# michael-fonder/M4Depth

Measured on AMD Instinct MI355X. Metric: frames/s, higher is better.
Workload: dtype f32

## Files before the change

### include/m4depth_hip.h

```cpp
#ifndef M4DEPTH_HIP_H_
#define M4DEPTH_HIP_H_

#include <stdint.h>

#ifdef __cplusplus
extern "C" {
#endif

#define M4D_ABI_VERSION 6

int m4d_abi_version(void);
long long m4d_launch_count(void);
const char* m4d_build_info(void);
const char* m4d_switches_info(void);


int m4d_backproject_fwd(const float* input, const float* coords, const int dims[6],
                        float* out, void* stream);

int m4d_backproject_bwd(const float* grad, const float* input, const float* coords,
                        const int dims[6], float* input_grad, float* coords_grad, void* stream);


int m4d_dense_image_warp(const float* image, const float* flow, int B, int H, int W, int C,
// ... 214 lines not shown
                    int b, int h, int w, int C, int nbre_cuts, int cv_accum,
                    float* f_input, int f_stride, float log_scale, void* stream);
int m4d_level_front_r(const float* raw_f, float* norm_out, const float* prev_f, const float* depth_prev_t,
                      const float* prev_l_parallax, const float* prev_l_other, int ph, int pw,
                      const float* rot, int rot_c, const float* trans, const float* cam_f, const float* cam_c,
                      int b, int h, int w, int C, int nbre_cuts, int dscv_range, int sncv_range, int cv_accum,
                      float* f_input, int f_stride, float log_scale, void* stream);

int m4d_camera_pyramid(const float* cam_f, const float* cam_c, int b, int levels, float* f_out, float* c_out,
                       void* stream);

int m4d_level_post(const float* refiner_out, const float* rot, int rot_c, const float* trans,
                   const float* cam_f, const float* cam_c, int b, int h, int w, float scale,
                   float* parallax, float* depth, float* other, float* depth_state, void* stream);

int m4d_bias_act(const float* x, const float* bias, long long rows, int C, float slope,
                 float* out, void* stream);

int m4d_bias_act_padded(const float* x, const float* bias, int b, int h, int w, int C, float slope,
                        float* out, int out_h, int out_w, int off_y, int off_x, void* stream);

int m4d_conv3x3_bias_act(const float* x, const float* wp, const float* bias, int b, int h, int w,
                         int Cin, int Cout, int CoutPad, float slope, float* out, void* stream);
long long m4d_conv3x3_workspace_floats(int b, int h, int w, int CoutPad);
int m4d_conv3x3s_bias_act_ws(const float* x, const float* wp, const float* bias, int b, int h, int w,
                             int Cin, int Cout, int CoutPad, int stride, float slope, float* out,
                             float* workspace, long long workspace_floats, void* stream);
int m4d_conv3x3_bias_act_ws(const float* x, const float* wp, const float* bias, int b, int h, int w,
                            int Cin, int Cout, int CoutPad, float slope, float* out, float* workspace,
                            long long workspace_floats, void* stream);
int m4d_conv3x3s_bias_act_wsb(const float* x, const float* wp, const float* bias, int b, int split_batch, int h, int w,
                              int Cin, int Cout, int CoutPad, int stride, float slope, float* out,
                              float* workspace, long long workspace_floats, void* stream);
int m4d_conv3x3_lat(const float* x, int s_in, long long x_slab_floats, const float* x_bias, float x_slope,
                    const void* wp, const float* bias, int b, int h, int w, int Cin, int Cout, float slope,
                    int mt, int kw, int s_out, float* out, long long out_slab_floats, void* stream);
int m4d_conv3x3s_lat(const float* x, int s_in, long long x_slab_floats, const float* x_bias, float x_slope,
                     const void* wp, const float* bias, int b, int h, int w, int Cin, int Cout, int stride, float slope,
                     int mt, int kw, int s_out, float* out, long long out_slab_floats, void* stream);
int m4d_conv3x3_lat_f16(const float* x, int s_in, long long x_slab_floats, const float* x_bias, float x_slope,
                        const void* wp, const float* bias, int b, int h, int w, int Cin, int Cout, float slope,
                        int mt, int kw, int s_out, float* out, long long out_slab_floats, void* stream);
int m4d_partial_finish(const float* x, int s_in, long long x_slab_floats, const float* bias, float slope,
                       long long pixels, int C, float* out, void* stream);

int m4d_conv3x3_small_bias_act(const float* x, const float* wp, const float* bias, int b, int h, int w,
                               int Cin, int Cout, int CoutPad, float slope, float* out, void* stream);
int m4d_conv3x3s_small_bias_act(const float* x, const float* wp, const float* bias, int b, int h, int w,
                                int Cin, int Cout, int CoutPad, int stride, float slope, float* out, void* stream);
int m4d_conv3x3_small6_bias_act(const float* x, const void* wp6, const float* bias, int b, int h, int w,
                                int Cin, int Cout, int CoutPad, float slope, float* out, void* stream);

long long m4d_dinl_workspace_floats(int b, int C);
int m4d_dinl_fwd_padded(const float* x, const float* scale, const float* bias, int b, int h, int w, int C,
                        float slope, float* workspace, float* out, int out_h, int out_w, int off_y,
                        int off_x, void* stream);
int m4d_dinl_fwd(const float* x, const float* scale, const float* bias, int b, int h, int w, int C,
                 float slope, float* workspace, float* out, void* stream);

int m4d_enc_level0_fwd(const float* images, int bsz, long long stride_b, long long stride_t,
                       const float* w1_hwio, const float* bias1, const float* dn_scale, const float* dn_bias,
                       float dn_slope, const float* w2_hwio, const float* bias2, float slope,
                       int b, int h, int w, float* workspace, float* out, void* stream);
int m4d_enc_level0_stats(const float* images, int bsz, long long stride_b, long long stride_t,
                         const float* w1_hwio, const float* bias1, int b, int h, int w, float* workspace,
                         float* mean, float* var, void* stream);
int m4d_enc_level0_apply(const float* images, int bsz, long long stride_b, long long stride_t,
                         const float* w1_hwio, const float* bias1, const float* mean, const float* var,
                         const float* dn_scale, const float* dn_bias, float dn_slope, const float* w2_hwio,
                         const float* bias2, float slope, int b, int h, int w, float* out, void* stream);
int m4d_enc_head_fwd(const float* images, int bsz, long long stride_b, long long stride_t,
                     const float* w_hwio, const float* bias, int b, int h, int w, int C,
                     float* workspace, float* raw_out, void* stream);
int m4d_conv3x3s2_dinl_bias_act(const float* x_raw, const float* mean, const float* var, const float* dn_scale,
                                const float* dn_bias, float dn_slope, const float* wp, const float* bias,
                                int b, int h, int w, int Cout, int CoutPad, float slope, float* out, void* stream);

long long m4d_metrics_workspace_bytes(void);
int m4d_depth_metrics(const float* gt, const float* est, long long n, float max_d, void* workspace,
                      float* out7, float* total7, float count, float* mean7, void* stream);
int m4d_depth_metrics_strided(const float* gt, long long per_image, long long gt_image_stride, const float* est,
                              long long n, float max_d, void* workspace, float* out7, float* total7, float count,
// ... 94 lines not shown
```

### m4depth_amd/csrc/m4d_conv.hip

```cpp
#include "m4d_common.h"
#include "../../include/m4depth_hip.h"

namespace {

typedef float f32x16 __attribute__((ext_vector_type(16)));

struct ConvArgs {
  const float* x; const float* wp; const float* bias; float* out;
  int b, h, w, Cin, Cout, CoutPad, n_chunks, tiles_x, tiles_y;
  int oh, ow, pad_y, pad_x;
  float slope;
  int ksplit, chunks_per_split;
  float* ws;
  const float* dn_mean; const float* dn_var; const float* dn_scale; const float* dn_bias; float dn_slope;
};

constexpr int kTW = 16, kTH = 8;
constexpr int kKC = 16, kRS = 20;

template <int NT, int TS, int STRIDE, bool DB, int MINB, bool DINL = false>
__global__ void __launch_bounds__(256, MINB)
conv3x3_mfma_kernel(const ConvArgs a) {
  constexpr int kHWT = (kTW - 1) * STRIDE + 3, kHHT = (kTH - 1) * STRIDE + 3, kHP = kHWT * kHHT;
  constexpr int BN = 32 * NT;
// ... 350 lines not shown
  __syncthreads();

  constexpr int kRP = 36;
  float* red = lds_dyn;
#pragma unroll
  for (int r = 0; r < 16; ++r) {
    const int mr = (r & 3) + 8 * (r >> 2) + 4 * kh;
    red[(wave * 32 + mr) * kRP + m] = acc[r];
  }
  __syncthreads();
  {
    const int p = t >> 3, cq = t & 7;
    const int oy = tile_y + (p >> 3), ox = tile_x + (p & 7);
    const int co = n0 + 4 * cq;
    if (oy < a.oh && ox < a.ow && co < a.Cout) {
      const float4 s0 = *reinterpret_cast<const float4*>(red + (0 * 32 + p) * kRP + 4 * cq);
      const float4 s1 = *reinterpret_cast<const float4*>(red + (1 * 32 + p) * kRP + 4 * cq);
      const float4 s2 = *reinterpret_cast<const float4*>(red + (2 * 32 + p) * kRP + 4 * cq);
      const float4 s3 = *reinterpret_cast<const float4*>(red + (3 * 32 + p) * kRP + 4 * cq);
      const float sum[4] = {((s0.x + s1.x) + s2.x) + s3.x, ((s0.y + s1.y) + s2.y) + s3.y,
                            ((s0.z + s1.z) + s2.z) + s3.z, ((s0.w + s1.w) + s2.w) + s3.w};
      float* op = a.out + (((long long)bi * a.oh + oy) * a.ow + ox) * a.Cout + co;
#pragma unroll
      for (int e = 0; e < 4; ++e) {
        if (co + e < a.Cout) {
          float v = sum[e] + a.bias[co + e];
          op[e] = v > 0.f ? v : v * a.slope;
        }
      }
    }
  }
}

typedef __bf16 s6_bf16x8 __attribute__((ext_vector_type(8)));
typedef __bf16 s6_bf16x2 __attribute__((ext_vector_type(2)));
constexpr int kS6Row = 24;
constexpr int kS6A = kSHP * kS6Row;
constexpr int kS6B = 9 * 32 * kS6Row;

__device__ __forceinline__ unsigned s6_pk(float a, float b) {
  s6_bf16x2 v; v[0] = (__bf16)a; v[1] = (__bf16)b;
  return __builtin_bit_cast(unsigned, v);
}

__global__ void __launch_bounds__(256, 1)
conv3x3_small6_kernel(const ConvArgs a) {
  constexpr int A_PER = (kSHP * 4 + 63) / 64;
  constexpr int B_PER = (9 * 32 * 6) / 64;
  extern __shared__ __align__(16) float lds_dyn[];
  const int t = threadIdx.x, lane = t & 63;
  const int wave = __builtin_amdgcn_readfirstlane(t >> 6);
  float* lds_a = lds_dyn + wave * (kS6A + kS6B);
  float* lds_b = lds_a + kS6A;
  const int tile = blockIdx.x;
  const int tile_y = (tile / a.tiles_x) * kSH, tile_x = (tile % a.tiles_x) * kSW;
  const int n0 = blockIdx.y * 32;
  const int bi = blockIdx.z;
  const float* ximg = a.x + (long long)bi * a.h * a.w * a.Cin;
  const unsigned char* wsplit = reinterpret_cast<const unsigned char*>(a.wp);

  int a_off[A_PER], a_dst[A_PER];
  unsigned a_ok = 0;
  const int aq = lane & 3;
#pragma unroll
  for (int u = 0; u < A_PER; ++u) {
    const int idx = u * 64 + lane;
// ... 149 lines not shown

template <int NT, int TS, int STRIDE, int MINB>
void launch_conv(const ConvArgs& a, dim3 grid, hipStream_t s) {
  constexpr bool DB = false;
  constexpr int HP = ((kTW - 1) * STRIDE + 3) * ((kTH - 1) * STRIDE + 3);
  constexpr size_t lds = (size_t)(HP * kRS + (DB ? 2 : 1) * TS * 32 * NT * kRS) * sizeof(float);
  if (lds > 64 * 1024) M4D_LDS_OPT_IN(&conv3x3_mfma_kernel<NT, TS, STRIDE, DB, MINB>);
  m4d_launch((conv3x3_mfma_kernel<NT, TS, STRIDE, DB, MINB>), grid, dim3(256), lds, s, a);
}

template <int STRIDE>
void dispatch_conv(const ConvArgs& a, int nt, dim3 grid, hipStream_t s) {
  const long long blocks = (long long)grid.x * grid.y * grid.z;
  constexpr long long occ3_min_blocks = 4 * 768;
  switch (nt) {
    case 4:
      if (STRIDE == 1 && blocks >= occ3_min_blocks) launch_conv<4, 3, STRIDE, STRIDE == 1 ? 3 : 1>(a, grid, s);
      else launch_conv<4, 3, STRIDE, STRIDE == 1 ? 2 : 1>(a, grid, s);
      break;
    case 3: launch_conv<3, 3, STRIDE, STRIDE == 1 ? 3 : 2>(a, grid, s); break;
    case 2: launch_conv<2, STRIDE == 1 ? 9 : 3, STRIDE, STRIDE == 1 ? 3 : 2>(a, grid, s); break;
    default: launch_conv<1, 9, STRIDE, STRIDE == 1 ? 4 : 2>(a, grid, s); break;
  }
}

}

extern "C" int m4d_conv3x3_bias_act(const float* x, const float* wp, const float* bias, int b, int h, int w,
                                    int Cin, int Cout, int CoutPad, float slope, float* out, void* stream) {
  return m4d_conv3x3s_bias_act_ws(x, wp, bias, b, h, w, Cin, Cout, CoutPad, 1, slope, out, nullptr, 0, stream);
}

static int launch_conv3x3_small(const float* x, const float* wp, const float* bias, int b, int h, int w, int Cin, int Cout,
                                int CoutPad, int stride, float slope, float* out, void* stream) {
  M4D_CHECK_ARG(x && wp && bias && out && b > 0 && h > 0 && w > 0 && Cout > 0 && (stride == 1 || stride == 2));
  M4D_CHECK_ARG(Cin >= 16 && Cin % 4 == 0 && CoutPad % 32 == 0 && CoutPad >= Cout);
  M4D_CHECK_ARG(((((uintptr_t)x) | ((uintptr_t)wp)) & 15u) == 0);
  ConvArgs a;
  a.x = x; a.wp = wp; a.bias = bias; a.out = out; a.b = b; a.h = h; a.w = w; a.Cin = Cin; a.Cout = Cout;
  a.CoutPad = CoutPad; a.n_chunks = (Cin + kKC - 1) / kKC;
  a.dn_mean = a.dn_var = a.dn_scale = a.dn_bias = nullptr; a.dn_slope = 1.0f;
  a.slope = slope;
  a.oh = (h + stride - 1) / stride; a.ow = (w + stride - 1) / stride;
  const int tot_y = (a.oh - 1) * stride + 3 - h, tot_x = (a.ow - 1) * stride + 3 - w;
  a.pad_y = (tot_y > 0 ? tot_y : 0) / 2; a.pad_x = (tot_x > 0 ? tot_x : 0) / 2;
  a.tiles_x = (a.ow + kSW - 1) / kSW; a.tiles_y = (a.oh + kSH - 1) / kSH;
  a.ksplit = 1; a.chunks_per_split = a.n_chunks; a.ws = nullptr;
  const int halo = ((kSW - 1) * stride + 3) * ((kSH - 1) * stride + 3);
  const size_t lds = (size_t)4 * (halo * kRS + kSB) * sizeof(float);
  if (stride == 1) M4D_LDS_OPT_IN(&conv3x3_small_kernel<1>);
  else M4D_LDS_OPT_IN(&conv3x3_small_kernel<2>);
  const dim3 grid((unsigned)(a.tiles_x * a.tiles_y), (unsigned)(CoutPad / 32), (unsigned)b);
  if (stride == 1) m4d_launch(conv3x3_small_kernel<1>, grid, dim3(256), lds, (hipStream_t)stream, a);
  else m4d_launch(conv3x3_small_kernel<2>, grid, dim3(256), lds, (hipStream_t)stream, a);
  return M4D_LAUNCH_RESULT();
}
extern "C" int m4d_conv3x3_small_bias_act(const float* x, const float* wp, const float* bias, int b, int h, int w,
                                          int Cin, int Cout, int CoutPad, float slope, float* out, void* stream) {
  return launch_conv3x3_small(x, wp, bias, b, h, w, Cin, Cout, CoutPad, 1, slope, out, stream);
}
extern "C" int m4d_conv3x3s_small_bias_act(const float* x, const float* wp, const float* bias, int b, int h, int w,
                                           int Cin, int Cout, int CoutPad, int stride, float slope, float* out, void* stream) {
  return launch_conv3x3_small(x, wp, bias, b, h, w, Cin, Cout, CoutPad, stride, slope, out, stream);
}

extern "C" int m4d_conv3x3_small6_bias_act(const float* x, const void* wp6, const float* bias, int b, int h, int w,
                                           int Cin, int Cout, int CoutPad, float slope, float* out, void* stream) {
  M4D_CHECK_ARG(x && wp6 && bias && out && b > 0 && h > 0 && w > 0 && Cout > 0);
  M4D_CHECK_ARG(Cin >= 16 && Cin % 4 == 0 && CoutPad % 32 == 0 && CoutPad >= Cout);
  M4D_CHECK_ARG(((((uintptr_t)x) | ((uintptr_t)wp6)) & 15u) == 0);
  ConvArgs a;
  a.x = x; a.wp = reinterpret_cast<const float*>(wp6); a.bias = bias; a.out = out; a.b = b; a.h = h; a.w = w; a.Cin = Cin; a.Cout = Cout;
  a.CoutPad = CoutPad; a.n_chunks = (Cin + kKC - 1) / kKC;
  a.dn_mean = a.dn_var = a.dn_scale = a.dn_bias = nullptr; a.dn_slope = 1.0f;
  a.oh = h; a.ow = w; a.pad_y = a.pad_x = 1; a.slope = slope;
  a.tiles_x = (w + kSW - 1) / kSW; a.tiles_y = (h + kSH - 1) / kSH;
  a.ksplit = 1; a.chunks_per_split = a.n_chunks; a.ws = nullptr;
  constexpr size_t lds = (size_t)4 * (kS6A + kS6B) * sizeof(float);
  M4D_LDS_OPT_IN(&conv3x3_small6_kernel);
  m4d_launch(conv3x3_small6_kernel, dim3((unsigned)(a.tiles_x * a.tiles_y), (unsigned)(CoutPad / 32), (unsigned)b), dim3(256),
                     lds, (hipStream_t)stream, a);
  return M4D_LAUNCH_RESULT();
}

extern "C" long long m4d_conv3x3_workspace_floats(int b, int h, int w, int CoutPad) {
  return 32LL * b * h * w * CoutPad;
}

extern "C" int m4d_conv3x3_bias_act_ws(const float* x, const float* wp, const float* bias, int b, int h, int w,
                                       int Cin, int Cout, int CoutPad, float slope, float* out, float* workspace,
                                       long long workspace_floats, void* stream) {
  return m4d_conv3x3s_bias_act_ws(x, wp, bias, b, h, w, Cin, Cout, CoutPad, 1, slope, out, workspace,
                                  workspace_floats, stream);
}

extern "C" int m4d_conv3x3s2_dinl_bias_act(const float* x_raw, const float* mean, const float* var, const float* dn_scale,
                                           const float* dn_bias, float dn_slope, const float* wp, const float* bias,
                                           int b, int h, int w, int Cout, int CoutPad, float slope, float* out, void* stream) {
  M4D_CHECK_ARG(x_raw && mean && var && dn_scale && dn_bias && wp && bias && out && b > 0 && h > 0 && w > 0 && Cout > 0);
  M4D_CHECK_ARG(CoutPad == 32 && Cout <= 32);
  M4D_CHECK_ARG(((((uintptr_t)x_raw) & 7u) == 0) && ((((uintptr_t)wp) & 15u) == 0));
  ConvArgs a;
  a.x = x_raw; a.wp = wp; a.bias = bias; a.out = out; a.b = b; a.h = h; a.w = w; a.Cin = 16; a.Cout = Cout;
  a.CoutPad = CoutPad; a.n_chunks = 1;
  a.oh = (h + 1) / 2; a.ow = (w + 1) / 2;
  const int tph = (a.oh - 1) * 2 + 3 - h, tpw = (a.ow - 1) * 2 + 3 - w;
  a.pad_y = (tph > 0 ? tph : 0) / 2; a.pad_x = (tpw > 0 ? tpw : 0) / 2;
  a.tiles_x = (a.ow + kTW - 1) / kTW; a.tiles_y = (a.oh + kTH - 1) / kTH; a.slope = slope;
  a.ksplit = 1; a.chunks_per_split = 1; a.ws = nullptr;
  a.dn_mean = mean; a.dn_var = var; a.dn_scale = dn_scale; a.dn_bias = dn_bias; a.dn_slope = dn_slope;
  constexpr int HP = ((kTW - 1) * 2 + 3) * ((kTH - 1) * 2 + 3);
  constexpr size_t lds = (size_t)(HP * kRS + 9 * 32 * kRS) * sizeof(float);
  if (lds > 64 * 1024) M4D_LDS_OPT_IN(&conv3x3_mfma_kernel<1, 9, 2, false, 2, true>);
  const dim3 grid((unsigned)(a.tiles_x * a.tiles_y), 1, (unsigned)b);
  m4d_launch((conv3x3_mfma_kernel<1, 9, 2, false, 2, true>), grid, dim3(256), lds, (hipStream_t)stream, a);
  return M4D_LAUNCH_RESULT();
}

extern "C" int m4d_conv3x3s_bias_act_wsb(const float* x, const float* wp, const float* bias, int b, int split_batch, int h,
                                         int w, int Cin, int Cout, int CoutPad, int stride, float slope, float* out,
                                         float* workspace, long long workspace_floats, void* stream);

extern "C" int m4d_conv3x3s_bias_act_ws(const float* x, const float* wp, const float* bias, int b, int h, int w,
                                        int Cin, int Cout, int CoutPad, int stride, float slope, float* out,
                                        float* workspace, long long workspace_floats, void* stream) {
  return m4d_conv3x3s_bias_act_wsb(x, wp, bias, b, b, h, w, Cin, Cout, CoutPad, stride, slope, out, workspace,
                                   workspace_floats, stream);
}

extern "C" int m4d_conv3x3s_bias_act_wsb(const float* x, const float* wp, const float* bias, int b, int split_batch, int h,
                                         int w, int Cin, int Cout, int CoutPad, int stride, float slope, float* out,
                                         float* workspace, long long workspace_floats, void* stream) {
  M4D_CHECK_ARG(x && wp && bias && out && b > 0 && split_batch > 0 && h > 0 && w > 0 && Cin > 0 && Cout > 0);
  M4D_CHECK_ARG((stride == 1 || stride == 2) && CoutPad % 32 == 0 && CoutPad >= Cout);
  M4D_CHECK_ARG(((((uintptr_t)x) & (Cin % 2 == 0 ? 7u : 3u)) == 0) && ((((uintptr_t)wp) & 15u) == 0));
  ConvArgs a;
  a.x = x; a.wp = wp; a.bias = bias; a.out = out; a.b = b; a.h = h; a.w = w; a.Cin = Cin; a.Cout = Cout;
  a.CoutPad = CoutPad; a.n_chunks = (Cin + kKC - 1) / kKC;
  a.dn_mean = a.dn_var = a.dn_scale = a.dn_bias = nullptr; a.dn_slope = 1.0f;
  a.oh = (h + stride - 1) / stride; a.ow = (w + stride - 1) / stride;
  const int tph = (a.oh - 1) * stride + 3 - h, tpw = (a.ow - 1) * stride + 3 - w;
  a.pad_y = (tph > 0 ? tph : 0) / 2; a.pad_x = (tpw > 0 ? tpw : 0) / 2;
  a.tiles_x = (a.ow + kTW - 1) / kTW; a.tiles_y = (a.oh + kTH - 1) / kTH; a.slope = slope;
  const long long tiles = (long long)a.tiles_x * a.tiles_y;
  const int n32 = CoutPad / 32;
  auto n_tiles_for = [&](int images) {
    int nt = n32 >= 4 && n32 % 4 == 0 ? 4 : (n32 % 3 == 0 ? 3 : (n32 % 2 == 0 ? 2 : 1));
    while (nt > 1 && tiles * images * (n32 / nt) < 512) nt = (nt == 4 || nt == 2) ? nt / 2 : 1;
    return nt;
  };
  const int nt = n_tiles_for(b);
  const long long blocks = tiles * split_batch * (n32 / n_tiles_for(split_batch));
  int ksplit = 1;
  constexpr int sk_target = 256, sk_min_chunks = 2, sk_max = 16;
  if (workspace != nullptr && blocks < 128 && a.n_chunks >= 4) {
    ksplit = (int)((sk_target + blocks - 1) / blocks);
    if (ksplit > a.n_chunks / sk_min_chunks) ksplit = a.n_chunks / sk_min_chunks;
    if (ksplit > sk_max) ksplit = sk_max;
    while (ksplit > 1 && (long long)ksplit * b * a.oh * a.ow * CoutPad > workspace_floats) --ksplit;
  }
  a.chunks_per_split = (a.n_chunks + ksplit - 1) / ksplit;
  ksplit = (a.n_chunks + a.chunks_per_split - 1) / a.chunks_per_split;
  a.ksplit = ksplit; a.ws = workspace;
  const dim3 grid((unsigned)tiles, (unsigned)(n32 / nt), (unsigned)(b * ksplit));
  hipStream_t s = (hipStream_t)stream;
  if (stride == 1) dispatch_conv<1>(a, nt, grid, s);
  else dispatch_conv<2>(a, nt, grid, s);
  if (ksplit > 1) {
    const long long pixels = (long long)b * a.oh * a.ow;
    long long g = (pixels * Cout + 255) / 256;
    if (g > 2048) g = 2048;
    m4d_launch(conv_splitk_reduce_kernel, dim3((unsigned)g), dim3(256), 0, s, workspace, bias, pixels, Cout,
                       CoutPad, ksplit, slope, out);
  }
  return M4D_LAUNCH_RESULT();
}
```

### m4depth_amd/network_ops.py

```python
from __future__ import annotations

import ctypes

import torch

from ._lib import lib, dptr, stream_ptr, check, as_f32
from .depth_operations import _CV_ACCUM


def normalize_cuts(x, nbre_cuts, out=None):
    x = as_f32(x, "x")
    b, h, w, C = x.shape
    if C % nbre_cuts != 0:
        raise ValueError(f"nbre_cuts={nbre_cuts} does not divide the {C} feature channels")
    if out is None:
        out = torch.empty_like(x)
    check(lib.m4d_normalize_cuts(dptr(x, "x"), b, h, w, C, int(nbre_cuts), dptr(out, "out"), stream_ptr()),
          "m4d_normalize_cuts")
    return out


def resize_bilinear_v1(x, out_h, out_w, mul=1.0):
    x = as_f32(x, "x")
    b, ih, iw, c = x.shape
    out = torch.empty((b, out_h, out_w, c), dtype=torch.float32, device=x.device)
    check(lib.m4d_resize_bilinear_v1(dptr(x, "x"), b, ih, iw, c, int(out_h), int(out_w), float(mul), dptr(out),
                                     stream_ptr()), "m4d_resize_bilinear_v1")
    return out


def resize_nearest(x, out_h, out_w, out=None):
    x = as_f32(x, "x")
    b, ih, iw, c = x.shape
    if out is None:
        out = torch.empty((b, out_h, out_w, c), dtype=torch.float32, device=x.device)
# ... 885 lines not shown
    est = as_f32(est, "est")
    b, h, w = est.shape[:3]
    if est.dim() != 4 or est.shape[3] != 1:
        raise ValueError(f"est: expected [b,h,w,1], got {tuple(est.shape)}")
    gs = _batch_stride(gt, "gt")
    if gt.shape[0] != b or gt.dim() not in (3, 4) or (gt.dim() == 4 and gt.shape[3] != 1):
        raise ValueError(f"gt {tuple(gt.shape)} is not the [b,H,W,1] ground truth of est {tuple(est.shape)}")
    H, W = gt.shape[1:3]
    if log.dim() != 2 or log.shape[1] != 2:
        raise ValueError(f"log: expected [rows, 2], got {tuple(log.shape)}")
    for name, t in (("counter", counter), ("first_bad", first_bad)):
        if not isinstance(t, torch.Tensor) or t.numel() != 1:
            raise ValueError(f"{name}: expected a one-element int64 device tensor")
    ws = _workspace("train_log", int(lib.m4d_train_log_workspace_bytes()), est.device)
    check(lib.m4d_train_log_step(dptr(loss.reshape(1), "loss"), ctypes.c_void_p(gt.data_ptr()), gs, dptr(est, "est"), b, H, W,
                                 h, w, dptr(log, "log"), log.shape[0], dptr(counter, "counter", torch.int64),
                                 dptr(first_bad, "first_bad", torch.int64), dptr(ws), stream_ptr()), "m4d_train_log_step")
    return log

def pack_conv_weights(kernel_hwio):
    import numpy as np
    k = np.asarray(kernel_hwio, dtype=np.float32)
    assert k.shape[:2] == (3, 3)
    cin, cout = k.shape[2], k.shape[3]
    nch = -(-cin // 16)
    cpad = -(-cout // 32) * 32
    full = np.zeros((3, 3, nch * 16, cpad), np.float32)
    full[:, :, :cin, :cout] = k
    perm = np.array([0, 2, 4, 6, 8, 10, 12, 14, 1, 3, 5, 7, 9, 11, 13, 15])
    w = full.reshape(9, nch, 16, cpad)[:, :, perm, :]
    return np.ascontiguousarray(w.transpose(1, 0, 3, 2)), cpad


def conv3x3_bias_act(x, wp, bias, cout, cout_pad, slope=0.1, stride=1, split_batch=None):
    x = as_f32(x, "x")
    b, h, w, cin = x.shape
    split_b = b if split_batch is None else int(split_batch)
    oh, ow = -(-h // stride), -(-w // stride)
    out = torch.empty((b, oh, ow, cout), dtype=torch.float32, device=x.device)
    ws = None
    ws_floats = 0
    if split_b * oh * ow <= 16384:
        ws_floats = int(lib.m4d_conv3x3_workspace_floats(b, oh, ow, int(cout_pad)))
        ws = _workspace("conv_splitk", 4 * ws_floats, x.device)
    if split_batch is None:
        check(lib.m4d_conv3x3s_bias_act_ws(dptr(x, "x"), dptr(wp, "wp"), dptr(bias, "bias"), b, h, w, cin, int(cout),
                                           int(cout_pad), int(stride), float(slope), dptr(out), dptr(ws), ws_floats,
                                           stream_ptr()), "m4d_conv3x3s_bias_act_ws")
    else:
        check(lib.m4d_conv3x3s_bias_act_wsb(dptr(x, "x"), dptr(wp, "wp"), dptr(bias, "bias"), b, split_b, h, w, cin, int(cout),
                                            int(cout_pad), int(stride), float(slope), dptr(out), dptr(ws), ws_floats,
                                            stream_ptr()), "m4d_conv3x3s_bias_act_wsb")
    return out


def conv3x3_small_bias_act(x, wp, bias, cout, cout_pad, slope=0.1, stride=1):
    x = as_f32(x, "x")
    b, h, w, cin = x.shape
    out = torch.empty((b, -(-h // stride), -(-w // stride), cout), dtype=torch.float32, device=x.device)
    check(lib.m4d_conv3x3s_small_bias_act(dptr(x, "x"), dptr(wp, "wp"), dptr(bias, "bias"), b, h, w, cin, int(cout),
                                          int(cout_pad), int(stride), float(slope), dptr(out), stream_ptr()),
          "m4d_conv3x3s_small_bias_act")
    return out


_WINO_G = [[1.0, 0.0, 0.0], [0.5, 0.5, 0.5], [0.5, -0.5, 0.5], [0.0, 0.0, 1.0]]


_WINO_SKEW = 64


def pack_conv_weights_winograd(kernel_hwio, chunk=16):
    import numpy as np
    k = np.asarray(kernel_hwio, dtype=np.float64)
    assert k.shape[:2] == (3, 3)
    cin, cout = k.shape[2], k.shape[3]
    G = np.array(_WINO_G, np.float64)
    U = np.einsum('ij,jkco,lk->ilco', G, k, G)
    nch = -(-cin // chunk)
    cpad = -(-cout // 32) * 32
    full = np.zeros((16, nch * chunk, cpad), np.float32)
    full[:, :cin, :cout] = U.reshape(16, cin, cout).astype(np.float32)
    w = np.ascontiguousarray(full.reshape(16, nch, chunk, cpad).transpose(1, 0, 3, 2))
    if chunk == 8:
        skewed = np.zeros((nch, 16, cpad * chunk + _WINO_SKEW), np.float32)
        skewed[:, :, :cpad * chunk] = w.reshape(nch, 16, cpad * chunk)
        return skewed, cpad
    return w, cpad


def conv3x3_wino_bias_act(x, wu, bias, cout, cout_pad, slope=0.1):
    x = as_f32(x, "x")
# ... 122 lines not shown
    return np.concatenate([w.reshape(-1), texp.astype(np.int16).view(np.uint16)])


class PartialAct:

    def __init__(self, slabs, bias, slope):
        self.slabs, self.bias, self.slope = slabs, bias, 1.0 if slope is None else float(slope)

    @property
    def shape(self):
        return self.slabs.shape[1:]

    @property
    def is_cuda(self):
        return self.slabs.is_cuda

    @property
    def device(self):
        return self.slabs.device

    def dense(self):
        S, b, h, w, C = self.slabs.shape
        out = torch.empty((b, h, w, C), dtype=torch.float32, device=self.slabs.device)
        check(lib.m4d_partial_finish(dptr(self.slabs, "slabs"), S, b * h * w * C, dptr(self.bias, "bias"), self.slope,
                                     b * h * w, C, dptr(out), stream_ptr()), "m4d_partial_finish")
        return out


def _lat_halo_pixels(mt, stride):
    mtx, mty = (2 if mt >= 4 else 1), (2 if mt >= 2 else 1)
    return ((8 * mtx - 1) * stride + 3) * ((4 * mty - 1) * stride + 3)


import os as _os
lat_max_workgroups = int(_os.environ.get("M4D_LAT_MAX_WG", "256"))


def lat_config(b, h, w, cin, cout, final=False, stride=1):
    n_chunks, n_groups = -(-cin // 16), -(-cout // 32)
    oh, ow = -(-h // stride), -(-w // stride)
    s_out = 1 if final else min(4, n_chunks)
    while s_out > 1 and (s_out - 1) * (-(-n_chunks // s_out)) >= n_chunks:
        s_out -= 1
    cps = -(-n_chunks // s_out)
    kw = 1 if cps <= 1 else (2 if cps <= 2 else 4)

    def wgs(mt, kw):
        mtx, mty = (2 if mt == 4 else 1), (2 if mt >= 2 else 1)
        tiles = b * (-(-oh // (4 * mty))) * (-(-ow // (8 * mtx)))
        return tiles * (-(-n_groups // (4 // kw))) * s_out

    def fits(mt, kw):
        return 2 * kw * _lat_halo_pixels(mt, stride) * 96 <= 160 * 1024
    mt = 1
    while (wgs(mt, kw) > lat_max_workgroups or not fits(mt, kw)) and kw > 1:
        kw //= 2
    while wgs(mt, kw) > lat_max_workgroups and mt < 4 and fits(mt * 2, kw):
        mt *= 2
    return mt, kw, s_out


def conv3x3_lat(x, wp, bias, cout, slope=0.1, final=False, config=None, stride=1):
    if isinstance(x, PartialAct):
        xs, s_in, x_bias, x_slope = x.slabs, x.slabs.shape[0], x.bias, x.slope
        b, h, w, cin = x.shape
        slab = b * h * w * cin
    else:
# ... 494 lines not shown
```

Measured before the change: 1811.

## Add dedicated stride-2 conv3x3 MFMA kernels with even/odd column-split LDS layout

Adds specialized stride-2 3x3 convolution kernels, one for the regular path and one for the small path. Both stage the input halo in LDS with even and odd columns split apart, so strided tap reads become contiguous. Both also prefetch the next chunk's weights and activations in registers during the MFMA loop. They become the default for stride-2 cases that meet the alignment, no-split-k and single-tile conditions, with an environment flag to fall back to the older kernels. The new paths add code and register pressure, and they may not beat the tuned generic template on every shape.

```diff
diff --git a/include/m4depth_hip.h b/include/m4depth_hip.h
--- a/include/m4depth_hip.h
+++ b/include/m4depth_hip.h
@@ -270,6 +270,9 @@
 int m4d_conv3x3s_bias_act_wsb(const float* x, const float* wp, const float* bias, int b, int split_batch, int h, int w,
                               int Cin, int Cout, int CoutPad, int stride, float slope, float* out,
                               float* workspace, long long workspace_floats, void* stream);
+int m4d_conv3x3s_bias_act_wsb_k(const float* x, const float* wp, const float* bias, int b, int split_batch, int h, int w,
+                                int Cin, int Cout, int CoutPad, int stride, float slope, float* out,
+                                float* workspace, long long workspace_floats, int kernel, void* stream);
 int m4d_conv3x3_lat(const float* x, int s_in, long long x_slab_floats, const float* x_bias, float x_slope,
                     const void* wp, const float* bias, int b, int h, int w, int Cin, int Cout, float slope,
                     int mt, int kw, int s_out, float* out, long long out_slab_floats, void* stream);
@@ -286,6 +289,8 @@
                                int Cin, int Cout, int CoutPad, float slope, float* out, void* stream);
 int m4d_conv3x3s_small_bias_act(const float* x, const float* wp, const float* bias, int b, int h, int w,
                                 int Cin, int Cout, int CoutPad, int stride, float slope, float* out, void* stream);
+int m4d_conv3x3s_small_bias_act_k(const float* x, const float* wp, const float* bias, int b, int h, int w,
+                                  int Cin, int Cout, int CoutPad, int stride, float slope, float* out, int kernel, void* stream);
 int m4d_conv3x3_small6_bias_act(const float* x, const void* wp6, const float* bias, int b, int h, int w,
                                 int Cin, int Cout, int CoutPad, float slope, float* out, void* stream);
 
diff --git a/m4depth_amd/csrc/m4d_conv.hip b/m4depth_amd/csrc/m4d_conv.hip
--- a/m4depth_amd/csrc/m4d_conv.hip
+++ b/m4depth_amd/csrc/m4d_conv.hip
@@ -406,6 +406,282 @@
   }
 }
 
+constexpr int kS2HW = (kTW - 1) * 2 + 3, kS2HH = (kTH - 1) * 2 + 3, kS2HP = kS2HW * kS2HH;
+constexpr int kS2Ev = (kS2HW + 1) / 2;
+constexpr int kS2Row = 672;
+constexpr int kS2SHW = (kSW - 1) * 2 + 3, kS2SHH = (kSH - 1) * 2 + 3, kS2SHP = kS2SHW * kS2SHH;
+constexpr int kS2SEv = (kS2SHW + 1) / 2;
+constexpr int kS2SRow = 368;
+constexpr int kS2SA = kS2SHH * kS2SRow;
+
+#define M4D_S2_LDS_BARRIER() do { asm volatile("s_waitcnt lgkmcnt(0)" ::: "memory"); __builtin_amdgcn_s_barrier(); asm volatile("" ::: "memory"); } while (0)
+
+__global__ void __launch_bounds__(256, 2)
+conv3x3_s2_kernel(const ConvArgs a) {
+  constexpr int A_PER = (kS2HP * 4 + 255) / 256;
+  extern __shared__ __align__(16) float lds_dyn[];
+  float* lds_a = lds_dyn;
+  const int t = threadIdx.x, lane = t & 63;
+  const int wave = __builtin_amdgcn_readfirstlane(t >> 6);
+  const int tile = blockIdx.x;
+  const int tile_y = (tile / a.tiles_x) * kTH, tile_x = (tile % a.tiles_x) * kTW;
+  const int n0 = blockIdx.y * 32;
+  const int bi = blockIdx.z;
+  const float* ximg = a.x + (long long)bi * a.h * a.w * a.Cin;
+
+  int a_off[A_PER], a_dst[A_PER];
+  unsigned a_ok = 0;
+  const int aq = t & 3;
+#pragma unroll
+  for (int u = 0; u < A_PER; ++u) {
+    const int idx = u * 256 + t;
+    const int hp = min(idx >> 2, kS2HP - 1);
+    const int hy = hp / kS2HW, hx = hp - hy * kS2HW;
+    const int gy = tile_y * 2 - a.pad_y + hy, gx = tile_x * 2 - a.pad_x + hx;
+    const bool ok = gy >= 0 && gy < a.h && gx >= 0 && gx < a.w;
+    a_ok |= ok ? (1u << u) : 0u;
+    a_off[u] = (min(max(gy, 0), a.h - 1) * a.w + min(max(gx, 0), a.w - 1)) * a.Cin + 4 * aq;
+    a_dst[u] = hy * kS2Row + ((hx & 1) * kS2Ev + (hx >> 1)) * kRS + 2 * aq;
+  }
+  const int m = lane & 31, kh = lane >> 5;
+  const float* w_lane = a.wp + (long long)(n0 + m) * kKC + kh * 8;
+  const long long w_tap = (long long)a.CoutPad * kKC;
+
+  float4 ra[A_PER], rn[A_PER], rb0[9], rb1[9];
+  auto load_a = [&](float4 (&r)[A_PER], int chunk) __attribute__((always_inline)) {
+    const int cc = min(chunk * kKC, a.Cin - 4 - 4 * aq);
+#pragma unroll
+    for (int u = 0; u < A_PER; ++u) r[u] = *reinterpret_cast<const float4*>(ximg + a_off[u] + cc);
+  };
+  auto commit_a = [&](const float4 (&r)[A_PER], int chunk) __attribute__((always_inline)) {
+    const bool ch_ok = chunk * kKC + 4 * aq < a.Cin;
+#pragma unroll
+    for (int u = 0; u < A_PER; ++u) {
+      const bool ok = ((a_ok >> u) & 1u) && ch_ok;
+      const float4 v = r[u];
+      *reinterpret_cast<float2*>(lds_a + a_dst[u]) = make_float2(ok ? v.x : 0.f, ok ? v.z : 0.f);
+      *reinterpret_cast<float2*>(lds_a + a_dst[u] + 8) = make_float2(ok ? v.y : 0.f, ok ? v.w : 0.f);
+    }
+  };
+  auto load_b = [&](int chunk) __attribute__((always_inline)) {
+    const float* wc = w_lane + chunk * 9 * w_tap;
+#pragma unroll
+    for (int tap = 0; tap < 9; ++tap) {
+      rb0[tap] = *reinterpret_cast<const float4*>(wc + tap * w_tap);
+      rb1[tap] = *reinterpret_cast<const float4*>(wc + tap * w_tap + 4);
+    }
+  };
+
+  f32x16 acc;
+#pragma unroll
+  for (int r = 0; r < 16; ++r) acc[r] = 0.f;
+  const int prow = 2 * wave + (m >> 4), pcol = m & 15;
+  const float* a_lane = lds_a + prow * 2 * kS2Row + pcol * kRS + kh * 8;
+  auto read_a = [&](int tap, float4& a0, float4& a1) __attribute__((always_inline)) {
+    const int ky = tap / 3, kx = tap % 3;
+    const float* ap = a_lane + ky * kS2Row + ((kx & 1) * kS2Ev + (kx >> 1)) * kRS;
+    a0 = *reinterpret_cast<const float4*>(ap); a1 = *reinterpret_cast<const float4*>(ap + 4);
+  };
+  auto compute_chunk = [&](auto mode_tag, int next) __attribute__((always_inline)) {
+    constexpr int MODE = decltype(mode_tag)::value;
+    const float* wn = w_lane + next * 9 * w_tap;
+    float4 fa[2][2];
+    read_a(0, fa[0][0], fa[0][1]);
+#pragma unroll
+    for (int tap = 0; tap < 9; ++tap) {
+      if (tap + 1 < 9) read_a(tap + 1, fa[(tap + 1) & 1][0], fa[(tap + 1) & 1][1]);
+      const float4 a0 = fa[tap & 1][0], a1 = fa[tap & 1][1];
+      const float av[8] = {a0.x, a0.y, a0.z, a0.w, a1.x, a1.y, a1.z, a1.w};
+      const float bv[8] = {rb0[tap].x, rb0[tap].y, rb0[tap].z, rb0[tap].w, rb1[tap].x, rb1[tap].y, rb1[tap].z, rb1[tap].w};
+#pragma unroll
+      for (int ks = 0; ks < 8; ++ks) acc = __builtin_amdgcn_mfma_f32_32x32x2f32(av[ks], bv[ks], acc, 0, 0, 0);
+      if (MODE >= 1) {
+        rb0[tap] = *reinterpret_cast<const float4*>(wn + tap * w_tap);
+        rb1[tap] = *reinterpret_cast<const float4*>(wn + tap * w_tap + 4);
+        if (MODE == 2 && tap == 0) load_a(rn, next);
+        __builtin_amdgcn_sched_barrier(0);
+      }
+    }
+  };
+
+  const int n = a.n_chunks;
+  const int co = n0 + m;
+  float bias = a.bias[min(co, a.Cout - 1)];
+  load_a(ra, 0);
+  load_b(0);
+  load_a(rn, min(1, n - 1));
+  commit_a(ra, 0);
+  asm volatile("" : "+v"(bias));
+  M4D_S2_LDS_BARRIER();
+  __builtin_amdgcn_sched_barrier(0);
+  if (n > 1) {
+    compute_chunk(m4d_int<1>{}, 1);
+    M4D_S2_LDS_BARRIER();
+    commit_a(rn, 1);
+    M4D_S2_LDS_BARRIER();
+    for (int c = 1; c + 1 < n; ++c) {
+      compute_chunk(m4d_int<2>{}, c + 1);
+      M4D_S2_LDS_BARRIER();
+      commit_a(rn, c + 1);
+      M4D_S2_LDS_BARRIER();
+    }
+  }
+  compute_chunk(m4d_int<0>{}, 0);
+
+  float* oimg = a.out + (long long)bi * a.oh * a.ow * a.Cout;
+#pragma unroll
+  for (int r = 0; r < 16; ++r) {
+    const int mr = (r & 3) + 8 * (r >> 2) + 4 * kh;
+    const int oy = tile_y + 2 * wave + (mr >> 4), ox = tile_x + (mr & 15);
+    if (co < a.Cout && oy < a.oh && ox < a.ow) {
+      float v = acc[r] + bias;
+      v = v > 0.f ? v : v * a.slope;
+      oimg[((long long)oy * a.ow + ox) * a.Cout + co] = v;
+    }
+  }
+}
+
+__global__ void __launch_bounds__(256, 2)
+conv3x3_small_s2_kernel(const ConvArgs a) {
+  constexpr int A_PER = (kS2SHP * 4 + 63) / 64;
+  extern __shared__ __align__(16) float lds_dyn[];
+  const int t = threadIdx.x, lane = t & 63;
+  const int wave = __builtin_amdgcn_readfirstlane(t >> 6);
+  float* lds_a = lds_dyn + wave * kS2SA;
+  const int tile = blockIdx.x;
+  const int tile_y = (tile / a.tiles_x) * kSH, tile_x = (tile % a.tiles_x) * kSW;
+  const int n0 = blockIdx.y * 32;
+  const int bi = blockIdx.z;
+  const float* ximg = a.x + (long long)bi * a.h * a.w * a.Cin;
+
+  int a_off[A_PER], a_dst[A_PER];
+  unsigned a_ok = 0;
+  const int aq = lane & 3;
+#pragma unroll
+  for (int u = 0; u < A_PER; ++u) {
+    const int idx = u * 64 + lane;
+    const int hp = min(idx >> 2, kS2SHP - 1);
+    const int hy = hp / kS2SHW, hx = hp - hy * kS2SHW;
+    const int gy = tile_y * 2 - a.pad_y + hy, gx = tile_x * 2 - a.pad_x + hx;
+    const bool ok = gy >= 0 && gy < a.h && gx >= 0 && gx < a.w;
+    a_ok |= ok ? (1u << u) : 0u;
+    a_off[u] = (min(max(gy, 0), a.h - 1) * a.w + min(max(gx, 0), a.w - 1)) * a.Cin + 4 * aq;
+    a_dst[u] = hy * kS2SRow + ((hx & 1) * kS2SEv + (hx >> 1)) * kRS + 2 * aq;
+  }
+  const int m = lane & 31, kh = lane >> 5;
+  const float* w_lane = a.wp + (long long)(n0 + m) * kKC + kh * 8;
+  const long long w_tap = (long long)a.CoutPad * kKC;
+
+  float4 ra[A_PER], rb0[9], rb1[9];
+  bool ra_ch_ok = true;
+  auto load_a = [&](int chunk) __attribute__((always_inline)) {
+    ra_ch_ok = chunk * kKC + 4 * aq < a.Cin;
+    const int cc = min(chunk * kKC, a.Cin - 4 - 4 * aq);
+#pragma unroll
+    for (int u = 0; u < A_PER; ++u) ra[u] = *reinterpret_cast<const float4*>(ximg + a_off[u] + cc);
+  };
+  auto commit_a = [&]() __attribute__((always_inline)) {
+#pragma unroll
+    for (int u = 0; u < A_PER; ++u) {
+      const bool ok = ((a_ok >> u) & 1u) && ra_ch_ok;
+      const float4 v = ra[u];
+      *reinterpret_cast<float2*>(lds_a + a_dst[u]) = make_float2(ok ? v.x : 0.f, ok ? v.z : 0.f);
+      *reinterpret_cast<float2*>(lds_a + a_dst[u] + 8) = make_float2(ok ? v.y : 0.f, ok ? v.w : 0.f);
+    }
+  };
+
+  f32x16 acc;
+#pragma unroll
+  for (int r = 0; r < 16; ++r) acc[r] = 0.f;
+  const float* a_lane = lds_a + (m >> 3) * 2 * kS2SRow + (m & 7) * kRS + kh * 8;
+  auto read_a = [&](int tap, float4& a0, float4& a1) __attribute__((always_inline)) {
+    const int ky = tap / 3, kx = tap % 3;
+    const float* ap = a_lane + ky * kS2SRow + ((kx & 1) * kS2SEv + (kx >> 1)) * kRS;
+    a0 = *reinterpret_cast<const float4*>(ap); a1 = *reinterpret_cast<const float4*>(ap + 4);
+  };
+  auto compute_chunk = [&](auto next_tag, int next) __attribute__((always_inline)) {
+    constexpr bool NEXT = decltype(next_tag)::value != 0;
+    const float* wn = w_lane + next * 9 * w_tap;
+    float4 fa[2][2];
+    read_a(0, fa[0][0], fa[0][1]);
+#pragma unroll
+    for (int tap = 0; tap < 9; ++tap) {
+      if (tap + 1 < 9) read_a(tap + 1, fa[(tap + 1) & 1][0], fa[(tap + 1) & 1][1]);
+      const float4 a0 = fa[tap & 1][0], a1 = fa[tap & 1][1];
+      const float av[8] = {a0.x, a0.y, a0.z, a0.w, a1.x, a1.y, a1.z, a1.w};
+      const float bv[8] = {rb0[tap].x, rb0[tap].y, rb0[tap].z, rb0[tap].w, rb1[tap].x, rb1[tap].y, rb1[tap].z, rb1[tap].w};
+#pragma unroll
+      for (int ks = 0; ks < 8; ++ks) acc = __builtin_amdgcn_mfma_f32_32x32x2f32(av[ks], bv[ks], acc, 0, 0, 0);
+      if (NEXT) {
+        rb0[tap] = *reinterpret_cast<const float4*>(wn + tap * w_tap);
+        rb1[tap] = *reinterpret_cast<const float4*>(wn + tap * w_tap + 4);
+        __builtin_amdgcn_sched_barrier(0);
+      }
+    }
+  };
+
+  float bq[4];
+#pragma unroll
+  for (int e = 0; e < 4; ++e) bq[e] = a.bias[min(n0 + 4 * (t & 7) + e, a.Cout - 1)];
+  if (wave < a.n_chunks) {
+    load_a(wave);
+    {
+      const float* wc = w_lane + wave * 9 * w_tap;
+#pragma unroll
+      for (int tap = 0; tap < 9; ++tap) {
+        rb0[tap] = *reinterpret_cast<const float4*>(wc + tap * w_tap);
+        rb1[tap] = *reinterpret_cast<const float4*>(wc + tap * w_tap + 4);
+      }
+    }
+    int c = wave;
+    for (; c + 4 < a.n_chunks; c += 4) {
+      commit_a();
+      __builtin_amdgcn_wave_barrier();
+      load_a(c + 4);
+      __builtin_amdgcn_sched_barrier(0);
+      compute_chunk(m4d_int<1>{}, c + 4);
+      __builtin_amdgcn_wave_barrier();
+    }
+    commit_a();
+    __builtin_amdgcn_wave_barrier();
+    compute_chunk(m4d_int<0>{}, 0);
+    __builtin_amdgcn_wave_barrier();
+  }
+#pragma unroll
+  for (int e = 0; e < 4; ++e) asm volatile("" : "+v"(bq[e]));
+  __syncthreads();
+
+  constexpr int kRP = 36;
+  float* red = lds_dyn;
+#pragma unroll
+  for (int r = 0; r < 16; ++r) {
+    const int mr = (r & 3) + 8 * (r >> 2) + 4 * kh;
+    red[(wave * 32 + mr) * kRP + m] = acc[r];
+  }
+  __syncthreads();
+  {
+    const int p = t >> 3, cq = t & 7;
+    const int oy = tile_y + (p >> 3), ox = tile_x + (p & 7);
+    const int co = n0 + 4 * cq;
+    if (oy < a.oh && ox < a.ow && co < a.Cout) {
+      const float4 s0 = *reinterpret_cast<const float4*>(red + (0 * 32 + p) * kRP + 4 * cq);
+      const float4 s1 = *reinterpret_cast<const float4*>(red + (1 * 32 + p) * kRP + 4 * cq);
+      const float4 s2 = *reinterpret_cast<const float4*>(red + (2 * 32 + p) * kRP + 4 * cq);
+      const float4 s3 = *reinterpret_cast<const float4*>(red + (3 * 32 + p) * kRP + 4 * cq);
+      const float sum[4] = {((s0.x + s1.x) + s2.x) + s3.x, ((s0.y + s1.y) + s2.y) + s3.y,
+                            ((s0.z + s1.z) + s2.z) + s3.z, ((s0.w + s1.w) + s2.w) + s3.w};
+      float* op = a.out + (((long long)bi * a.oh + oy) * a.ow + ox) * a.Cout + co;
+#pragma unroll
+      for (int e = 0; e < 4; ++e) {
+        if (co + e < a.Cout) {
+          float v = sum[e] + bq[e];
+          op[e] = v > 0.f ? v : v * a.slope;
+        }
+      }
+    }
+  }
+}
+
 typedef __bf16 s6_bf16x8 __attribute__((ext_vector_type(8)));
 typedef __bf16 s6_bf16x2 __attribute__((ext_vector_type(2)));
 constexpr int kS6Row = 24;
@@ -621,8 +897,9 @@
 }
 
 static int launch_conv3x3_small(const float* x, const float* wp, const float* bias, int b, int h, int w, int Cin, int Cout,
-                                int CoutPad, int stride, float slope, float* out, void* stream) {
+                                int CoutPad, int stride, float slope, float* out, int kernel, void* stream) {
   M4D_CHECK_ARG(x && wp && bias && out && b > 0 && h > 0 && w > 0 && Cout > 0 && (stride == 1 || stride == 2));
+  M4D_CHECK_ARG(kernel == 0 || kernel == 1);
   M4D_CHECK_ARG(Cin >= 16 && Cin % 4 == 0 && CoutPad % 32 == 0 && CoutPad >= Cout);
   M4D_CHECK_ARG(((((uintptr_t)x) | ((uintptr_t)wp)) & 15u) == 0);
   ConvArgs a;
@@ -635,6 +912,11 @@
   a.pad_y = (tot_y > 0 ? tot_y : 0) / 2; a.pad_x = (tot_x > 0 ? tot_x : 0) / 2;
   a.tiles_x = (a.ow + kSW - 1) / kSW; a.tiles_y = (a.oh + kSH - 1) / kSH;
   a.ksplit = 1; a.chunks_per_split = a.n_chunks; a.ws = nullptr;
+  if (kernel == 0 && stride == 2 && (long long)h * w * Cin < (1LL << 31)) {
+    const dim3 grid2((unsigned)(a.tiles_x * a.tiles_y), (unsigned)(CoutPad / 32), (unsigned)b);
+    m4d_launch(conv3x3_small_s2_kernel, grid2, dim3(256), (size_t)4 * kS2SA * sizeof(float), (hipStream_t)stream, a);
+    return M4D_LAUNCH_RESULT();
+  }
   const int halo = ((kSW - 1) * stride + 3) * ((kSH - 1) * stride + 3);
   const size_t lds = (size_t)4 * (halo * kRS + kSB) * sizeof(float);
   if (stride == 1) M4D_LDS_OPT_IN(&conv3x3_small_kernel<1>);
@@ -646,11 +928,16 @@
 }
 extern "C" int m4d_conv3x3_small_bias_act(const float* x, const float* wp, const float* bias, int b, int h, int w,
                                           int Cin, int Cout, int CoutPad, float slope, float* out, void* stream) {
-  return launch_conv3x3_small(x, wp, bias, b, h, w, Cin, Cout, CoutPad, 1, slope, out, stream);
+  return launch_conv3x3_small(x, wp, bias, b, h, w, Cin, Cout, CoutPad, 1, slope, out, 0, stream);
 }
 extern "C" int m4d_conv3x3s_small_bias_act(const float* x, const float* wp, const float* bias, int b, int h, int w,
                                            int Cin, int Cout, int CoutPad, int stride, float slope, float* out, void* stream) {
-  return launch_conv3x3_small(x, wp, bias, b, h, w, Cin, Cout, CoutPad, stride, slope, out, stream);
+  return launch_conv3x3_small(x, wp, bias, b, h, w, Cin, Cout, CoutPad, stride, slope, out, 0, stream);
+}
+extern "C" int m4d_conv3x3s_small_bias_act_k(const float* x, const float* wp, const float* bias, int b, int h, int w,
+                                             int Cin, int Cout, int CoutPad, int stride, float slope, float* out, int kernel,
+                                             void* stream) {
+  return launch_conv3x3_small(x, wp, bias, b, h, w, Cin, Cout, CoutPad, stride, slope, out, kernel, stream);
 }
 
 extern "C" int m4d_conv3x3_small6_bias_act(const float* x, const void* wp6, const float* bias, int b, int h, int w,
@@ -706,20 +993,28 @@
   return M4D_LAUNCH_RESULT();
 }
 
-extern "C" int m4d_conv3x3s_bias_act_wsb(const float* x, const float* wp, const float* bias, int b, int split_batch, int h,
-                                         int w, int Cin, int Cout, int CoutPad, int stride, float slope, float* out,
-                                         float* workspace, long long workspace_floats, void* stream);
+extern "C" int m4d_conv3x3s_bias_act_wsb_k(const float* x, const float* wp, const float* bias, int b, int split_batch, int h,
+                                           int w, int Cin, int Cout, int CoutPad, int stride, float slope, float* out,
+                                           float* workspace, long long workspace_floats, int kernel, void* stream);
 
 extern "C" int m4d_conv3x3s_bias_act_ws(const float* x, const float* wp, const float* bias, int b, int h, int w,
                                         int Cin, int Cout, int CoutPad, int stride, float slope, float* out,
                                         float* workspace, long long workspace_floats, void* stream) {
-  return m4d_conv3x3s_bias_act_wsb(x, wp, bias, b, b, h, w, Cin, Cout, CoutPad, stride, slope, out, workspace,
-                                   workspace_floats, stream);
+  return m4d_conv3x3s_bias_act_wsb_k(x, wp, bias, b, b, h, w, Cin, Cout, CoutPad, stride, slope, out, workspace,
+                                     workspace_floats, 0, stream);
 }
 
 extern "C" int m4d_conv3x3s_bias_act_wsb(const float* x, const float* wp, const float* bias, int b, int split_batch, int h,
                                          int w, int Cin, int Cout, int CoutPad, int stride, float slope, float* out,
                                          float* workspace, long long workspace_floats, void* stream) {
+  return m4d_conv3x3s_bias_act_wsb_k(x, wp, bias, b, split_batch, h, w, Cin, Cout, CoutPad, stride, slope, out, workspace,
+                                     workspace_floats, 0, stream);
+}
+
+extern "C" int m4d_conv3x3s_bias_act_wsb_k(const float* x, const float* wp, const float* bias, int b, int split_batch, int h,
+                                           int w, int Cin, int Cout, int CoutPad, int stride, float slope, float* out,
+                                           float* workspace, long long workspace_floats, int kernel, void* stream) {
+  M4D_CHECK_ARG(kernel == 0 || kernel == 1);
   M4D_CHECK_ARG(x && wp && bias && out && b > 0 && split_batch > 0 && h > 0 && w > 0 && Cin > 0 && Cout > 0);
   M4D_CHECK_ARG((stride == 1 || stride == 2) && CoutPad % 32 == 0 && CoutPad >= Cout);
   M4D_CHECK_ARG(((((uintptr_t)x) & (Cin % 2 == 0 ? 7u : 3u)) == 0) && ((((uintptr_t)wp) & 15u) == 0));
@@ -753,7 +1048,10 @@
   a.ksplit = ksplit; a.ws = workspace;
   const dim3 grid((unsigned)tiles, (unsigned)(n32 / nt), (unsigned)(b * ksplit));
   hipStream_t s = (hipStream_t)stream;
-  if (stride == 1) dispatch_conv<1>(a, nt, grid, s);
+  if (kernel == 0 && stride == 2 && nt == 1 && ksplit == 1 && Cin % 4 == 0 && (((uintptr_t)x) & 15u) == 0 &&
+      (long long)h * w * Cin < (1LL << 31))
+    m4d_launch(conv3x3_s2_kernel, grid, dim3(256), (size_t)kS2HH * kS2Row * sizeof(float), s, a);
+  else if (stride == 1) dispatch_conv<1>(a, nt, grid, s);
   else dispatch_conv<2>(a, nt, grid, s);
   if (ksplit > 1) {
     const long long pixels = (long long)b * a.oh * a.ow;
diff --git a/m4depth_amd/network_ops.py b/m4depth_amd/network_ops.py
--- a/m4depth_amd/network_ops.py
+++ b/m4depth_amd/network_ops.py
@@ -1,6 +1,7 @@
 from __future__ import annotations
 
 import ctypes
+import os as _os
 
 import torch
 
@@ -952,6 +953,9 @@
     return np.ascontiguousarray(w.transpose(1, 0, 3, 2)), cpad
 
 
+conv_s2_legacy = _os.environ.get("M4D_CONV_S2_LEGACY", "0") == "1"
+
+
 def conv3x3_bias_act(x, wp, bias, cout, cout_pad, slope=0.1, stride=1, split_batch=None):
     x = as_f32(x, "x")
     b, h, w, cin = x.shape
@@ -963,7 +967,11 @@
     if split_b * oh * ow <= 16384:
         ws_floats = int(lib.m4d_conv3x3_workspace_floats(b, oh, ow, int(cout_pad)))
         ws = _workspace("conv_splitk", 4 * ws_floats, x.device)
-    if split_batch is None:
+    if conv_s2_legacy and stride == 2:
+        check(lib.m4d_conv3x3s_bias_act_wsb_k(dptr(x, "x"), dptr(wp, "wp"), dptr(bias, "bias"), b, split_b, h, w, cin, int(cout),
+                                              int(cout_pad), int(stride), float(slope), dptr(out), dptr(ws), ws_floats, 1,
+                                              stream_ptr()), "m4d_conv3x3s_bias_act_wsb_k")
+    elif split_batch is None:
         check(lib.m4d_conv3x3s_bias_act_ws(dptr(x, "x"), dptr(wp, "wp"), dptr(bias, "bias"), b, h, w, cin, int(cout),
                                            int(cout_pad), int(stride), float(slope), dptr(out), dptr(ws), ws_floats,
                                            stream_ptr()), "m4d_conv3x3s_bias_act_ws")
@@ -978,6 +986,11 @@
     x = as_f32(x, "x")
     b, h, w, cin = x.shape
     out = torch.empty((b, -(-h // stride), -(-w // stride), cout), dtype=torch.float32, device=x.device)
+    if conv_s2_legacy and stride == 2:
+        check(lib.m4d_conv3x3s_small_bias_act_k(dptr(x, "x"), dptr(wp, "wp"), dptr(bias, "bias"), b, h, w, cin, int(cout),
+                                                int(cout_pad), int(stride), float(slope), dptr(out), 1, stream_ptr()),
+              "m4d_conv3x3s_small_bias_act_k")
+        return out
     check(lib.m4d_conv3x3s_small_bias_act(dptr(x, "x"), dptr(wp, "wp"), dptr(bias, "bias"), b, h, w, cin, int(cout),
                                           int(cout_pad), int(stride), float(slope), dptr(out), stream_ptr()),
           "m4d_conv3x3s_small_bias_act")
@@ -1166,7 +1179,6 @@
     return ((8 * mtx - 1) * stride + 3) * ((4 * mty - 1) * stride + 3)
 
 
-import os as _os
 lat_max_workgroups = int(_os.environ.get("M4D_LAT_MAX_WG", "256"))
 
 
```

After: 1826, median of 6. About the same (+0.8%).
